# venetanji/videosd

Measured on AMD Instinct MI355X. Metric: frames/sec (whole node) + p50 per-frame latency, SD1.5 512x512 LCM 4-step, higher is better.
Workload: dtype f16 (fp32 accumulate); 1 GPU; 5 frames per launch x 4 launch lanes in flight (a stream's independent frames coalesced along GEMM M; the batch=1-per-launch figures of a --full run are fps_one_frame_per_launch and p50_latency_ms) of SD1.5 512x512 LCM 4-step img2img, every frame denoised independently, ControlNet-canny + TAESD (BASELINE configs[1], reference-faithful: the reference always runs ControlNet); frames_per_rank=414, frames_per_launch=5, launches_in_flight_per_gpu=4, kernel_launches_per_graph_replay=1430

## Files before the change

include/vsd.h:

```cpp
#ifndef VSD_H
#define VSD_H
#include <stdint.h>

#ifdef __cplusplus
extern "C" {
#endif

typedef struct vsd_ctx vsd_ctx;

enum vsd_status {
  VSD_OK = 0,
  VSD_ERR_ARG = -1,
  VSD_ERR_HIP = -2,
  VSD_ERR_NOMEM = -3,
  VSD_ERR_STATE = -4,
  VSD_PLAN_OTHER_PROGRAM = 1
};

enum vsd_act { VSD_ACT_NONE = 0, VSD_ACT_RELU = 1, VSD_ACT_SILU = 2, VSD_ACT_GEGLU = 3, VSD_ACT_QUICKGELU = 4,
               VSD_ACT_SOFTMAX = 5 ,
               VSD_ACT_GELU = 6 ,
               VSD_ACT_POST = 256  };

enum vsd_tile { VSD_TILE_128x128 = 0, VSD_TILE_128x64 = 1, VSD_TILE_64x64 = 2, VSD_TILE_64x128 = 3,
                VSD_TILE_256x128 = 4 ,
                VSD_TILE_256x64 = 5 ,
                VSD_TILE_256x256 = 6  };

enum vsd_family {
  VSD_FAM_CONV_GEMM = 0, VSD_FAM_SPLITK_REDUCE = 1, VSD_FAM_GROUPNORM = 2, VSD_FAM_LAYERNORM = 3,
  VSD_FAM_ATTENTION = 4, VSD_FAM_ELEMENTWISE = 5, VSD_FAM_COUNT = 6
};

#define VSD_VERSION 10
int vsd_version(void);
int vsd_conv_desc_size(void);

vsd_ctx* vsd_create(int device_id);
void vsd_destroy(vsd_ctx* ctx);
const char* vsd_last_error(vsd_ctx* ctx);

typedef struct vsd_conv_desc {
  const void* src0;
  const void* src1;
  int32_t c0, c1;
  int32_t hs, ws;
  int32_t hi, wi;
  int32_t ho, wo;
  int32_t ksize, stride, pad;
  const void* weight;
  int32_t n, k, kp;
  const void* bias;
  const void* rowvec;
  const void* residual;
  const void* residual2;
  int32_t ldr;
  float out_scale;
  int32_t act;
  void* out;
  int32_t ldo;
  void* out2;
  const void* add2;
  void* out_t;
  int32_t ldt, t_col0;
  int32_t tile;
  int32_t split_k;
  void* workspace;
  int32_t pipeline;
  void* rowstat_out;
  void* chanstat_out;
  void* chanstat_part;
  void* chan_counters;
  const void* ln_part;
  int32_t ln_groups;
  float ln_eps;
  const void* ln_s;
  const void* ln_t;
  void* counters;
  int32_t batch;
  int32_t t_img;
// ... 162 lines not shown
```

videosd_amd/csrc/conv_gemm.hip:

```cpp
#include "conv_kernels.h"


#ifdef VSD_CONV_PROBE
extern "C" void vsd_conv_set_probe(void* buf) { g_conv_probe = (long long*)buf; }
#endif
#ifdef VSD_WG_TIMELINE
extern "C" void vsd_wgtl_set(void* buf, int64_t words) { g_wgtl = (unsigned long long*)buf; g_wgtl_cap = (size_t)words; g_wgtl_off = 0; }
extern "C" int64_t vsd_wgtl_used(void) { return (int64_t)g_wgtl_off; }
extern "C" void vsd_cut_set(void* buf) { g_cut = (unsigned long long*)buf; }
#endif

struct ConvLaunch {
  ConvParams p;
  int BM, BN, grid, stages;
  bool halo, c64;
};

static int conv_setup(vsd_ctx* ctx, const vsd_conv_desc* d, ConvLaunch& cl, bool grouped) {
  ConvParams& p = cl.p;
  p.src0 = (const half_t*)d->src0;
  p.src1 = (const half_t*)d->src1;
  p.c0 = d->c0;
  p.c1 = d->src1 ? d->c1 : 0;
  p.cin = p.c0 + p.c1;
// ... 55 lines not shown
#endif
  p.rowstat_out = (float*)d->rowstat_out;
  p.chanstat_part = (float*)d->chanstat_part;
  p.chanstat_out = (float*)d->chanstat_out;
  p.chan_counters = (int*)d->chan_counters;
  p.ln_part = (const float*)d->ln_part;
  p.ln_groups = d->ln_groups;
  p.ln_eps = d->ln_eps;
  p.ln_s = (const float*)d->ln_s;
  p.ln_t = (const float*)d->ln_t;
  VSD_CUT_SET(p)
  const int stages = d->pipeline;
  if (stages != 0 && (stages < 3 || stages > 10)) return vsd_fail(ctx, VSD_ERR_ARG, "conv_gemm: pipeline %d (0, 3..10)", stages);
  if ((stages == 8 || stages == 9) && !p.fast)
    return vsd_fail(ctx, VSD_ERR_ARG, "conv_gemm: the eight-wave forms (pipelines 8, 9) exist for the buffer-load path only (Cin %% 64 == 0 per "
                    "source, no resize)");
  const bool c64 = stages == 10;
  const bool halo = stages == 7 || c64;

  if (!p.src0 || !p.w || !p.out) return vsd_fail(ctx, VSD_ERR_ARG, "conv_gemm: null src/weight/out");
  if (p.M <= 0 || p.N <= 0) return vsd_fail(ctx, VSD_ERR_ARG, "conv_gemm: empty problem M=%d N=%d", p.M, p.N);
  if (p.c0 % 8 || p.c1 % 8) return vsd_fail(ctx, VSD_ERR_ARG, "conv_gemm: channels must be multiples of 8 (%d,%d)", p.c0, p.c1);
  if (p.c1 && (p.c0 % 64 || p.c1 % 64)) return vsd_fail(ctx, VSD_ERR_ARG, "conv_gemm: concat sources need C %% 64 == 0");
  if (p.K != p.ksize * p.ksize * p.cin) return vsd_fail(ctx, VSD_ERR_ARG, "conv_gemm: K=%d != ks^2*Cin=%d", p.K, p.ksize * p.ksize * p.cin);
  if (p.Kp % BK || p.Kp < p.K) return vsd_fail(ctx, VSD_ERR_ARG, "conv_gemm: Kp=%d must be K rounded up to 64", p.Kp);
  if (p.ksize != 1 && p.ksize != 3) return vsd_fail(ctx, VSD_ERR_ARG, "conv_gemm: ksize %d", p.ksize);
  if (p.ldo % 8 || (p.residual && p.ldr % 8)) return vsd_fail(ctx, VSD_ERR_ARG, "conv_gemm: ld must be a multiple of 8");
  if (p.batch > 1 && p.chanstat_out) return vsd_fail(ctx, VSD_ERR_ARG, "conv_gemm: chanstat_out is per tensor, not per image (batch must be 1)");
  if (p.out_t && p.batch > 1 && (p.t_img < p.hw_out || (int64_t)p.batch * p.t_img > p.ldt))
    return vsd_fail(ctx, VSD_ERR_ARG, "conv_gemm: transposed output needs hw <= t_img and batch * t_img <= ldt");
  if (p.out2 && !p.add2) return vsd_fail(ctx, VSD_ERR_ARG, "conv_gemm: out2 without add2");
  if ((p.act & 0xff) > VSD_ACT_GELU) return vsd_fail(ctx, VSD_ERR_ARG, "conv_gemm: activation %d", p.act & 0xff);
  if ((p.act & 0xff) == VSD_ACT_GELU && (p.out_t || p.rowstat_out || p.ln_part || (p.act & VSD_ACT_POST)))
    return vsd_fail(ctx, VSD_ERR_ARG, "conv_gemm: erf GELU exists in the general epilogue walk only (no transposed output, row statistics, "
                    "fused LayerNorm or post-residual form)");
  if (p.rowstat_out && (p.N % 64 || p.out_t || (p.split_k > 1 && !d->counters)))
    return vsd_fail(ctx, VSD_ERR_ARG, "conv_gemm: rowstat_out needs N %% 64 == 0, no transposed output and the in-kernel split-K form");
  if (p.chanstat_out && (!p.chanstat_part || !p.chan_counters || p.N % 8 || p.out_t || (p.act & 0xff) == VSD_ACT_GEGLU ||
                         (p.split_k > 1 && !d->counters)))
    return vsd_fail(ctx, VSD_ERR_ARG, "conv_gemm: chanstat_out needs chanstat_part + chan_counters, N %% 8 == 0, a plain (non-transposed, "
                    "non-GEGLU) output and the in-kernel split-K form");
  if (p.ln_part && (p.ksize != 1 || !p.ln_s || !p.ln_t || p.ln_groups <= 0 || p.bias))
    return vsd_fail(ctx, VSD_ERR_ARG, "conv_gemm: fused LayerNorm needs a 1x1 layer, ln_s/ln_t and no separate bias");
  if (p.split_k > 1 && !p.ws_partial) return vsd_fail(ctx, VSD_ERR_ARG, "conv_gemm: split_k needs a workspace");
  int BM, BN;
  switch (d->tile) {
    case VSD_TILE_128x128: BM = 128; BN = 128; break;
    case VSD_TILE_128x64: BM = 128; BN = 64; break;
    case VSD_TILE_64x64: BM = 64; BN = 64; break;
    case VSD_TILE_64x128: BM = 64; BN = 128; break;
    case VSD_TILE_256x128: BM = 256; BN = 128; break;
    case VSD_TILE_256x64: BM = 256; BN = 64; break;
    case VSD_TILE_256x256: BM = 256; BN = 256; break;
    default: return vsd_fail(ctx, VSD_ERR_ARG, "conv_gemm: tile %d", d->tile);
  }
  if (halo) {
    const bool simple_epi = !p.out2 && !p.residual2 && !p.out_t && !p.rowstat_out && !p.chanstat_out && !p.ln_part &&
                            p.out_scale == 1.0f && !p.out_scale_dev &&
                            ((p.act & 0xff) == VSD_ACT_NONE || (p.act & 0xff) == VSD_ACT_RELU || (p.act & 0xff) == VSD_ACT_SILU) &&
                            !((p.act & VSD_ACT_POST) && (p.act & 0xff) != VSD_ACT_RELU);
    if (!p.halo_ok || p.ksize != 3 || p.stride != 1 || p.pad != 1 || BM < 128 || (p.N % 8 && !c64) || p.c0 % 64 || p.c1 % 64 || !simple_epi)
      return vsd_fail(ctx, VSD_ERR_ARG, "conv_gemm: the halo-patch form (pipeline 7) needs a 3x3 stride-1 conv, Cin %% 64 == 0 per "
                      "source, a 128- or 256-row tile and the plain epilogue");
  }
  if (c64) {
    const bool thin = p.N <= 8 && p.ldo == 8 && !p.residual && !(p.act & VSD_ACT_POST);
    if ((p.N != 64 && !thin) || p.cin != 64 || p.c1 != 0 || BM != 256 || BN != 64 || p.split_k != 1 || p.ldo % 8 || (size_t)p.M * p.ldo * 2 >= 0x7fffffffull)
      return vsd_fail(ctx, VSD_ERR_ARG, "conv_gemm: the persistent 64-channel form (pipeline 10) needs Cin = 64 from one source, Cout = 64 (or Cout <= 8 "
                      "with ldo = 8, no residual), tile 256x64, no split over K and an output below 2 GB");
  }
  if (BN == 256 && (stages < 8 || p.split_k != 1 || p.chanstat_out))
    return vsd_fail(ctx, VSD_ERR_ARG, "conv_gemm: the 256x256 tile exists on eight waves (pipeline 8 or 9), unsplit and without fused channel "
                    "statistics (its epilogue runs in row bands)");
  if (!halo && BM == 256 && BN != 256 && (BN != 128 || !p.fast || (stages != 3 && stages != 5 && stages < 8)))
    return vsd_fail(ctx, VSD_ERR_ARG, "conv_gemm: the 256x128 tile exists for the buffer-load path (Cin %% 64 == 0, no resize) "
                    "with the 3-stage ring (pipeline 3, 5, 8 or 9) only");
  if ((stages == 8 || stages == 9) && BM * BN < 128 * 128)
    return vsd_fail(ctx, VSD_ERR_ARG, "conv_gemm: the eight-wave forms (pipelines 8, 9) exist for tiles of 128 x 128 and larger");
  if ((p.act & 0xff) == VSD_ACT_GEGLU) {
    if (BN % 128 || p.N % 128 || p.split_k != 1 || (!p.bias && !p.ln_part) || p.out_t)
      return vsd_fail(ctx, VSD_ERR_ARG, "conv_gemm: GEGLU needs BN=128 or 256, N %% 128 == 0, bias, no split-K");
  }
  if ((p.act & 0xff) == VSD_ACT_SOFTMAX) {
    if (BN != 128 || halo || p.N % 128 || (p.split_k != 1 && !d->counters) || p.out_t || p.out2 || p.residual || p.rowstat_out || p.chanstat_out ||
        p.softmax_cols < 1 || p.softmax_cols > 128 || p.ldo % 8)
      return vsd_fail(ctx, VSD_ERR_ARG, "conv_gemm: the softmax epilogue needs BN=128, N %% 128 == 0, split-K only in the in-kernel form, a plain output and "
                      "1 <= softmax_cols <= 128");
  }
  if (p.out_t && (p.t_col0 % BN)) return vsd_fail(ctx, VSD_ERR_ARG, "conv_gemm: t_col0 must be a multiple of BN");
  p.tiles_m = halo ? p.batch * cdiv(p.ho, BM / 16) * cdiv(p.wo, 16) : cdiv(p.M, BM);
  p.tiles_n = cdiv(p.N, BN);
  const int KT = halo ? p.cin / BK : p.Kp / BK;
  if (p.split_k > KT) p.split_k = KT;
  p.kt_per_split = cdiv(KT, p.split_k);
  p.split_k = cdiv(KT, p.kt_per_split);
  if (p.split_k == 1) p.counters = nullptr;
  if (p.counters && p.tiles_m * p.tiles_n > VSD_SPLITK_MAX_TILES)
    return vsd_fail(ctx, VSD_ERR_ARG, "conv_gemm: %d tiles exceed the split-K counter buffer", p.tiles_m * p.tiles_n);
  const int grid = p.tiles_m * p.tiles_n * p.split_k;
  {
    const double a_bytes = (double)p.batch * p.img_in * p.cin * 2.0, w_bytes = (double)p.N * p.Kp * 2.0;
    const int G = p.tiles_n * p.split_k;
    const int gx = cdiv(G, 8);
    const int nslice = p.split_k < gx ? p.split_k : gx;
    const double by_w = w_bytes + a_bytes * (G < 8 ? G : 8) * nslice / (double)p.split_k;
    const double by_a = a_bytes + w_bytes * (p.tiles_m < 8 ? p.tiles_m : 8);
    const bool ok24 = p.tiles_m % 2 == 0 && G % 4 == 0, ok42 = p.tiles_m % 4 == 0 && G % 2 == 0;
    const double by_24 = ok24 ? 4.0 * a_bytes + 2.0 * w_bytes : 1e300, by_42 = ok42 ? 2.0 * a_bytes + 4.0 * w_bytes : 1e300;
    const char* force = getenv("VSD_CONV_ORDER");
    const bool no_grid = force && force[0] == '1' && force[1] == 'd';
    p.order = by_a < by_w ? 1 : 0;
    double best = by_a < by_w ? by_a : by_w;
    if (!no_grid && by_24 < best) { p.order = 2; best = by_24; }
    if (!no_grid && by_42 < best) { p.order = 3; best = by_42; }
    if (force && !no_grid) {
      const int f = atoi(force);
      if (f <= 1 || (f == 2 && ok24) || (f == 3 && ok42)) p.order = f;
// ... 116 lines not shown
```

videosd_amd/csrc/conv_halo.hip:

```cpp
#include "conv_kernels.h"

namespace {

__device__ __forceinline__ void splitk_reduce_body(const ConvParams& p) {
  VSD_CUT(VSD_CUT_REDUCE, p.cut)
  const int nch = (p.N + 7) / 8;
  const size_t total = (size_t)p.M * nch;
  const size_t slab = (size_t)p.M * p.N;
  for (size_t q = (size_t)blockIdx.x * 256 + threadIdx.x; q < total; q += (size_t)gridDim.x * 256) {
    int m = (int)(q / nch);
    int n = (int)(q - (size_t)m * nch) * 8;
    float v[8] = {0, 0, 0, 0, 0, 0, 0, 0};
    const float* s = p.ws_partial + (size_t)m * p.N + n;
    const bool full = n + 8 <= p.N;
    const bool transposed = p.out_t && n >= p.t_col0;
    const bool pre_res = full && p.residual != nullptr && !transposed;
    const bool pre_brv = false;
    const bool pre_raw = full && !p.ln_part;
    half8 rres = (half8){0, 0, 0, 0, 0, 0, 0, 0}, braw = rres, rvraw = rres;
    if (full) {
      constexpr int NB = 8;
      f32x4 lo[NB], hi[NB];
#pragma unroll
      for (int k = 0; k < NB; ++k) {
// ... 13 lines not shown
            v[4 + i] += hi[k][i];
          }
        }
      for (int k0 = NB; k0 < p.split_k; k0 += NB) {
#pragma unroll
        for (int k = 0; k < NB; ++k) {
          const int kk = k0 + k < p.split_k ? k0 + k : 0;
          lo[k] = *reinterpret_cast<const f32x4*>(s + kk * slab);
          hi[k] = *reinterpret_cast<const f32x4*>(s + kk * slab + 4);
        }
#pragma unroll
        for (int k = 0; k < NB; ++k)
          if (k0 + k < p.split_k) {
#pragma unroll
            for (int i = 0; i < 4; ++i) {
              v[i] += lo[k][i];
              v[4 + i] += hi[k][i];
            }
          }
      }
    } else {
      for (int k = 0; k < p.split_k; ++k) {
#pragma unroll
        for (int i = 0; i < 8; ++i)
          if (n + i < p.N) v[i] += s[k * slab + i];
      }
    }
    if (p.ln_part) {
      float mean, rstd;
      ln_row_stats(p, m, mean, rstd);
      ln_transform8(p, n, mean, rstd, v);
    }
    float rs = 0.f, rq = 0.f;
    const f32x4 z4 = (f32x4){0.f, 0.f, 0.f, 0.f};
    epilogue_store8(p, m, n, v, rs, rq, pre_res, rres, pre_brv, z4, z4, pre_raw, braw, rvraw);
  }
}
__global__ __launch_bounds__(256) void splitk_reduce_kernel(const ConvParams p) { splitk_reduce_body(p); }
__global__ __launch_bounds__(256) void splitk_reduce_group_kernel(const ConvGroup g) {
  const ConvParams& p = g.p[blockIdx.y];
  if (p.split_k <= 1 || p.counters) return;
  splitk_reduce_body(p);
}

template <int BN, int WMN, int NSB>
__global__ __launch_bounds__(128 * WMN) void conv_halo_kernel(const ConvParams p) {
  VSD_CUT(VSD_CUT_CONV_HALO, p.cut)
  prefetch_kernargs();
  WGTL_START()
  constexpr int NW = 2 * WMN, NT = 64 * NW;
  constexpr int BM = 64 * WMN, PW = 16, PH = 4 * WMN, HW_ = PW + 2;
  constexpr int HUSED = (PH + 2) * HW_;
  constexpr int HROWS = (HUSED + 8 * NW - 1) / (8 * NW) * (8 * NW);
  constexpr int AI = HROWS / (8 * NW), BR = BN / (8 * NW);
  static_assert(BR >= 1, "tile too narrow for this many waves");
  constexpr int TM = 64, TN = BN / 2, FM = TM / 16, FN = TN / 16;
  constexpr int BNP = BN + 4;
  constexpr int A_HALFS = HROWS * BK, B_HALFS = BN * BK;
  constexpr int STAGE_BYTES = (2 * A_HALFS + NSB * B_HALFS) * 2;
  constexpr int EPI_BYTES = BM * BNP * 4;
  constexpr int LDS_BYTES = STAGE_BYTES > EPI_BYTES ? STAGE_BYTES : EPI_BYTES;
  __shared__ __attribute__((aligned(16))) unsigned char smem[LDS_BYTES];
  half_t* Abuf = reinterpret_cast<half_t*>(smem);
  half_t* Bbuf = Abuf + 2 * A_HALFS;
  typedef __attribute__((address_space(3))) void* lds_ptr_t;
  constexpr int OOB = (int)0x80000000;

  const int tid = threadIdx.x, lane = tid & 63, wave = tid >> 6;
  const int wave_s = __builtin_amdgcn_readfirstlane(wave);
  const int wm = wave >> 1, wn = wave & 1;
  const int fr = lane & 15, fq = lane >> 4;

  int tile_m, grp;
  block_to_tile(p, blockIdx.x, tile_m, grp);
  const int split = fdiv(grp, p.fd_tiles_n);
  const int tile_n = grp - split * p.tiles_n;
  const int n0 = tile_n * BN;
  const int ppr = (p.wo + PW - 1) / PW, tpi = ((p.ho + PH - 1) / PH) * ppr;
  const int img = fdiv(tile_m, p.fd_tpi), trem = tile_m - img * tpi;
  const int prow = fdiv(trem, p.fd_ppr);
  const int y0 = prow * PH, x0 = (trem - prow * ppr) * PW;
  const int pix0 = img * p.img_in;
  const int opix0 = img * p.hw_out;
  auto row_ok = [&](int r) { return y0 + (r >> 4) < p.ho && x0 + (r & 15) < p.wo; };
  auto row_m = [&](int r) { return opix0 + (y0 + (r >> 4)) * p.wo + x0 + (r & 15); };

  const int ncb_all = p.cin / BK;
  const int cb_begin = split * p.kt_per_split;
  const int cb_end = min(ncb_all, cb_begin + p.kt_per_split);
  const int T = (cb_end - cb_begin) * 9;

  int apx[AI], alc[AI];
#pragma unroll
  for (int q = 0; q < AI; ++q) {
    const int row = 8 * (wave + NW * q) + (lane >> 3);
    const int hy = row / HW_, hx = row - hy * HW_;
    const int y = y0 - 1 + hy, x = x0 - 1 + hx;
    const bool in = row < HUSED && (unsigned)y < (unsigned)p.hi && (unsigned)x < (unsigned)p.wi;
    const int sy = (int)(((unsigned)y * p.rmul_y) >> p.rshift), sx = (int)(((unsigned)x * p.rmul_x) >> p.rshift);
    apx[q] = in ? pix0 + sy * p.ws + sx : -1;
    alc[q] = (((lane & 7) ^ (row & 7)) << 4);
  }
  int bvoff[BR];
#pragma unroll
  for (int i = 0; i < BR; ++i) {
    const int r = 8 * (wave + NW * i) + (lane >> 3);
    const int n = n0 + r;
    bvoff[i] = n < p.N ? n * p.Kp * 2 + (((lane & 7) ^ (r & 7)) << 4) : OOB;
  }
  const int anr0 = (int)((size_t)p.batch * p.img_in * p.c0 * 2), anr1 = (int)((size_t)p.batch * p.img_in * p.c1 * 2);
  const int bnr = (int)((size_t)p.N * p.Kp * 2);

#define HALO_ISSUE_A(CB_, BUF_)                                                                         \
  {                                                                                                     \
    const int ch_ = (CB_) * BK;                                                                         \
    const bool second_ = ch_ >= p.c0;                                                                   \
    const int cs2_ = (second_ ? p.c1 : p.c0) * 2;                                                       \
    const int soff_ = (second_ ? ch_ - p.c0 : ch_) * 2;                                                 \
    const __amdgpu_buffer_rsrc_t rs_ =                                                                  \
        __builtin_amdgcn_make_buffer_rsrc((void*)(second_ ? p.src1 : p.src0), 0, second_ ? anr1 : anr0, 0x00020000); \
    half_t* dst_ = Abuf + (BUF_) * A_HALFS;                                                             \
    _Pragma("unroll") for (int q = 0; q < AI; ++q) {                                                    \
      const int vo_ = apx[q] >= 0 ? __mul24(apx[q], cs2_) + alc[q] : OOB;                               \
      __builtin_amdgcn_raw_ptr_buffer_load_lds(rs_, (lds_ptr_t)(dst_ + 8 * (wave_s + NW * q) * BK), 16, vo_, soff_, 0, 0); \
    }                                                                                                   \
  }
                     \
#define HALO_ISSUE_A_PIECE(CB_, BUF_, Q_)                                                               \
  {                                                                                                     \
    const int ch_ = (CB_) * BK;                                                                         \
    const bool second_ = ch_ >= p.c0;                                                                   \
    const int cs2_ = (second_ ? p.c1 : p.c0) * 2;                                                       \
    const int soff_ = (second_ ? ch_ - p.c0 : ch_) * 2;                                                 \
    const __amdgpu_buffer_rsrc_t rs_ =                                                                  \
        __builtin_amdgcn_make_buffer_rsrc((void*)(second_ ? p.src1 : p.src0), 0, second_ ? anr1 : anr0, 0x00020000); \
    half_t* dst_ = Abuf + (BUF_) * A_HALFS;                                                             \
    int apx_ = apx[0], alc_ = alc[0];                                                                   \
    _Pragma("unroll") for (int q = 1; q < AI; ++q)                                                      \
      if (q == (Q_)) {                                                                                  \
        apx_ = apx[q];                                                                                  \
        alc_ = alc[q];                                                                                  \
      }                                                                                                 \
    const int vo_ = apx_ >= 0 ? __mul24(apx_, cs2_) + alc_ : OOB;                                       \
    __builtin_amdgcn_raw_ptr_buffer_load_lds(rs_, (lds_ptr_t)(dst_ + 8 * (wave_s + NW * (Q_)) * BK), 16, vo_, soff_, 0, 0); \
  }
#define HALO_ISSUE_B(TAP_, CB_, SLOT_)                                                                  \
  {                                                                                                     \
    const int soff_ = ((TAP_) * p.cin + (CB_) * BK) * 2;                                                \
    const __amdgpu_buffer_rsrc_t rsb_ = __builtin_amdgcn_make_buffer_rsrc((void*)p.w, 0, bnr, 0x00020000); \
    half_t* dst_ = Bbuf + (SLOT_) * B_HALFS;                                                            \
    _Pragma("unroll") for (int i = 0; i < BR; ++i) {                                                    \
      const int bv_ = bvoff[i] + 0;                                                                     \
      __builtin_amdgcn_raw_ptr_buffer_load_lds(rsb_, (lds_ptr_t)(dst_ + 8 * (wave_s + NW * i) * BK), 16, bv_, soff_, 0, 0); \
    }                                                                                                   \
  }

#ifdef VSD_CONV_PROBE
  long long pacc[8] = {0, 0, 0, 0, 0, 0, 0, 0};
  long long plast = __builtin_readcyclecounter();
#endif
  f32x4 acc[FM][FN];
#pragma unroll
  for (int i = 0; i < FM; ++i)
#pragma unroll
    for (int j = 0; j < FN; ++j) acc[i][j] = (f32x4){0.f, 0.f, 0.f, 0.f};

  int hr0[FM];
#pragma unroll
  for (int i = 0; i < FM; ++i) hr0[i] = (wm * (TM / PW) + i) * HW_ + fr;

  if (T > 0) {
    HALO_ISSUE_A(cb_begin, 0)
#pragma unroll
    for (int st = 0; st < NSB - 1; ++st)
      if (st < T) HALO_ISSUE_B(st % 9, cb_begin + st / 9, st)
  }
  constexpr int LEAD = NSB - 1;
  int tap = 0, cb = cb_begin, slot = 0;
  int tap2 = LEAD % 9, cb2 = cb_begin + LEAD / 9;
  int hist = 0;
  CPROBE(0)
  for (int t = 0; t < T; ++t) {
    const int later_b = min(LEAD - 1, T - 1 - t) * BR;
    const int nwait = later_b + __builtin_popcount(hist & ((1 << LEAD) - 1));
    if (nwait >= (LEAD - 1) * BR + LEAD) asm volatile("s_waitcnt vmcnt(%0)" ::"n"((LEAD - 1) * BR + LEAD) : "memory");
    else if (nwait >= (LEAD - 1) * BR + 1) asm volatile("s_waitcnt vmcnt(%0)" ::"n"((LEAD - 1) * BR + 1) : "memory");
    else if (nwait >= (LEAD - 1) * BR) asm volatile("s_waitcnt vmcnt(%0)" ::"n"((LEAD - 1) * BR) : "memory");
    else if (nwait >= BR) asm volatile("s_waitcnt vmcnt(%0)" ::"n"(BR) : "memory");
    else asm volatile("s_waitcnt vmcnt(0)" ::: "memory");
    CPROBE(1)
    __builtin_amdgcn_s_barrier();
    CPROBE(2)
    if (t + LEAD < T) {
      int ns = slot + LEAD;
      if (ns >= NSB) ns -= NSB;
      HALO_ISSUE_B(tap2, cb2, ns)
    }
    hist <<= 1;
    if (tap < AI && cb + 1 < cb_end) {
      HALO_ISSUE_A_PIECE(cb + 1, (cb + 1 - cb_begin) & 1, tap)
      hist |= 1;
    }
    CPROBE(3)
    const half_t* a = Abuf + ((cb - cb_begin) & 1) * A_HALFS;
    const half_t* b = Bbuf + slot * B_HALFS;
    const int ky = tap / 3, kx = tap - ky * 3;
    const int toff = ky * HW_ + kx;
    half8 af[2][FM], bf[2][FN];
#pragma unroll
    for (int i = 0; i < FM; ++i) {
      const int hr = hr0[i] + toff;
      const half_t* row = a + hr * BK;
      const int sw = hr & 7;
      af[0][i] = *reinterpret_cast<const half8*>(row + ((fq ^ sw) << 3));
      af[1][i] = *reinterpret_cast<const half8*>(row + (((4 + fq) ^ sw) << 3));
    }
#pragma unroll
    for (int j = 0; j < FN; ++j) {
      const int r = wn * TN + j * 16 + fr;
      const half_t* row = b + r * BK;
      bf[0][j] = *reinterpret_cast<const half8*>(row + ((fq ^ (r & 7)) << 3));
      bf[1][j] = *reinterpret_cast<const half8*>(row + (((4 + fq) ^ (r & 7)) << 3));
    }
#pragma unroll
    for (int ks = 0; ks < 2; ++ks)
#pragma unroll
      for (int i = 0; i < FM; ++i)
#pragma unroll
        for (int j = 0; j < FN; ++j) acc[i][j] = __builtin_amdgcn_mfma_f32_16x16x32_f16(af[ks][i], bf[ks][j], acc[i][j], 0, 0, 0);
    CPROBE(4)
    if (++slot == NSB) slot = 0;
    if (++tap == 9) { tap = 0; ++cb; }
    if (++tap2 == 9) { tap2 = 0; ++cb2; }
  }
#undef HALO_ISSUE_A
#undef HALO_ISSUE_A_PIECE
#undef HALO_ISSUE_B
  __syncthreads();
  WGTL_LOOP()

  constexpr int CH = BN / 8;
  constexpr int NIT = BM * CH / NT;
  half8 rpre[NIT];
  float brv[8], brv2[8];
  const int pre_n = n0 + (tid % CH) * 8;
  const bool ncol_ok = pre_n + 8 <= p.N;
#pragma unroll
  for (int i = 0; i < 8; ++i) brv[i] = brv2[i] = 0.f;
  if (p.split_k == 1) {
    if (ncol_ok && p.bias) {
      half8 v = *reinterpret_cast<const half8*>(p.bias + pre_n);
#pragma unroll
      for (int i = 0; i < 8; ++i) brv[i] += (float)v[i];
    }
    if (ncol_ok && p.rowvec) {
      half8 v = *reinterpret_cast<const half8*>(p.rowvec + pre_n);
#pragma unroll
      for (int i = 0; i < 8; ++i) brv[i] += (float)v[i];
    }
    if (p.residual) {
#pragma unroll
      for (int j = 0; j < NIT; ++j) {
        const int q = tid + j * NT;
        const int r = q / CH;
        rpre[j] = *reinterpret_cast<const half8*>(p.residual + (ncol_ok && row_ok(r) ? (size_t)row_m(r) * p.ldr + pre_n : 0));
      }
    }
  }
  float* Cs = reinterpret_cast<float*>(smem);
#pragma unroll
  for (int i = 0; i < FM; ++i)
#pragma unroll
    for (int j = 0; j < FN; ++j) {
      const int col = wn * TN + j * 16 + fr;
      const int row = wm * TM + i * 16 + fq * 4;
#pragma unroll
      for (int r = 0; r < 4; ++r) Cs[(row + r) * BNP + col] = acc[i][j][r];
    }
  __syncthreads();
  CPROBE(5)
  bool from_slabs = false;
  if (p.split_k > 1) {
    float* slab = p.ws_partial + (size_t)split * p.M * p.N;
    const bool wt = p.counters != nullptr;
    __amdgpu_buffer_rsrc_t rsrc = __builtin_amdgcn_make_buffer_rsrc(
        slab, 0, (int)min((size_t)p.M * p.N * sizeof(float), (size_t)0x7fffffff), 0x00020000);
#pragma unroll
    for (int j = 0; j < NIT; ++j) {
      const int q = tid + j * NT;
      const int r = q / CH, c8 = (q - r * CH) * 8;
      const int n = n0 + c8;
      if (n + 8 <= p.N && row_ok(r)) {
        const float* sp = Cs + r * BNP + c8;
        if (wt) {
          const int off = (int)(((size_t)row_m(r) * p.N + n) * sizeof(float));
          __builtin_amdgcn_raw_buffer_store_b128(*reinterpret_cast<const u32x4*>(sp), rsrc, off, 0, 16);
          __builtin_amdgcn_raw_buffer_store_b128(*reinterpret_cast<const u32x4*>(sp + 4), rsrc, off + 16, 0, 16);
        } else {
          float* d = slab + (size_t)row_m(r) * p.N + n;
          *reinterpret_cast<f32x4*>(d) = *reinterpret_cast<const f32x4*>(sp);
          *reinterpret_cast<f32x4*>(d + 4) = *reinterpret_cast<const f32x4*>(sp + 4);
        }
      }
    }
    if (!p.counters) { WGTL_END(1) return; }
    asm volatile("s_waitcnt vmcnt(0)" ::: "memory");
    __syncthreads();
    int* lastflag = reinterpret_cast<int*>(smem);
    if (tid == 0) {
      int* cnt = p.counters + tile_n * p.tiles_m + tile_m;
      const int ticket = __hip_atomic_fetch_add(cnt, 1, __ATOMIC_RELAXED, __HIP_MEMORY_SCOPE_AGENT);
      const int last = ticket == p.split_k - 1;
      if (last) {
        __builtin_amdgcn_fence(__ATOMIC_ACQUIRE, "agent");
        asm volatile("s_waitcnt vmcnt(0)" ::: "memory");
        __hip_atomic_store(cnt, 0, __ATOMIC_RELAXED, __HIP_MEMORY_SCOPE_AGENT);
      }
      *lastflag = last;
    }
    __syncthreads();
    if (!*lastflag) { WGTL_END(1) return; }
    from_slabs = true;
    if (ncol_ok && p.bias) {
      half8 v = *reinterpret_cast<const half8*>(p.bias + pre_n);
#pragma unroll
      for (int i = 0; i < 8; ++i) brv[i] += (float)v[i];
    }
    if (ncol_ok && p.rowvec) {
      half8 v = *reinterpret_cast<const half8*>(p.rowvec + pre_n);
#pragma unroll
      for (int i = 0; i < 8; ++i) brv2[i] = (float)v[i];
    }
    if (p.residual) {
#pragma unroll
      for (int j = 0; j < NIT; ++j) {
        const int q = tid + j * NT;
        const int r = q / CH;
        rpre[j] = *reinterpret_cast<const half8*>(p.residual + (ncol_ok && row_ok(r) ? (size_t)row_m(r) * p.ldr + pre_n : 0));
      }
    }
  }
  const int act = p.act & 0xff;
  const bool post = (p.act & VSD_ACT_POST) != 0;
  auto finish = [&](auto act_tag) __attribute__((always_inline)) {
    constexpr int ACT = decltype(act_tag)::value;
#pragma unroll
    for (int j = 0; j < NIT; ++j) {
      const int q = tid + j * NT;
      const int r = q / CH, c8 = (q - r * CH) * 8;
      const int n = n0 + c8;
      if (n + 8 <= p.N && row_ok(r)) {
        f32x4 lo, hi;
        if (from_slabs) {
          lo = hi = (f32x4){0.f, 0.f, 0.f, 0.f};
          const float* sp = p.ws_partial + (size_t)row_m(r) * p.N + n;
          const size_t slab_sz = (size_t)p.M * p.N;
          constexpr int NB = 8;
          for (int k0 = 0; k0 < p.split_k; k0 += NB) {
            f32x4 a[NB], b[NB];
#pragma unroll
            for (int k = 0; k < NB; ++k) {
              const int kk = k0 + k < p.split_k ? k0 + k : 0;
              a[k] = *reinterpret_cast<const f32x4*>(sp + kk * slab_sz);
              b[k] = *reinterpret_cast<const f32x4*>(sp + kk * slab_sz + 4);
            }
#pragma unroll
            for (int k = 0; k < NB; ++k)
              if (k0 + k < p.split_k) {
#pragma unroll
                for (int i = 0; i < 4; ++i) {
                  lo[i] += a[k][i];
                  hi[i] += b[k][i];
                }
              }
          }
        } else {
          lo = *reinterpret_cast<const f32x4*>(Cs + r * BNP + c8);
          hi = *reinterpret_cast<const f32x4*>(Cs + r * BNP + c8 + 4);
        }
        const float v[8] = {lo[0], lo[1], lo[2], lo[3], hi[0], hi[1], hi[2], hi[3]};
        half8 o;
#pragma unroll
        for (int i = 0; i < 8; ++i) {
          float x = (v[i] + brv[i]) + brv2[i];
          if (ACT == 1) x = fmaxf(x, 0.f);
          if (ACT == 2) x = silu_f(x);
          if (p.residual) x += (float)rpre[j][i];
          if (ACT == 3) x = fmaxf(x, 0.f);
          o[i] = (half_t)x;
        }
        VSD_OUT_STORE8(p.out + (size_t)row_m(r) * p.ldo + n, o);
      }
    }
  };
  if (act == VSD_ACT_RELU && post) finish(std::integral_constant<int, 3>{});
  else if (act == VSD_ACT_RELU) finish(std::integral_constant<int, 1>{});
  else if (act == VSD_ACT_SILU) finish(std::integral_constant<int, 2>{});
  else finish(std::integral_constant<int, 0>{});
  CPROBE(6)
  CPROBE_OUT()
  WGTL_END(1)
}

}

void vsd_launch_conv_halo(const ConvParams& p, int BM, int BN, int grid, hipStream_t s) {
  if (BM == 256 && BN == 128) hipLaunchKernelGGL((conv_halo_kernel<128, 4, 3>), dim3(grid), dim3(512), 0, s, p);
  else if (BM == 256) hipLaunchKernelGGL((conv_halo_kernel<64, 4, 3>), dim3(grid), dim3(512), 0, s, p);
  else if (BN == 128) hipLaunchKernelGGL((conv_halo_kernel<128, 2, 3>), dim3(grid), dim3(256), 0, s, p);
  else hipLaunchKernelGGL((conv_halo_kernel<64, 2, 3>), dim3(grid), dim3(256), 0, s, p);
}

void vsd_launch_splitk_reduce(const ConvParams& p, int grid, hipStream_t s) {
  hipLaunchKernelGGL(splitk_reduce_kernel, dim3(grid), dim3(256), 0, s, p);
}
void vsd_launch_splitk_reduce_group(const ConvGroup& g, int grid, hipStream_t s) {
  hipLaunchKernelGGL(splitk_reduce_group_kernel, dim3(grid, g.n), dim3(256), 0, s, g);
}
```

videosd_amd/lib.py:

```python
import ctypes as C
import os

HERE = os.path.dirname(os.path.abspath(__file__))
LIB_PATH = os.environ.get("VSD_LIB") or os.path.join(HERE, "libvsd.so")

VERSION = 10
ACT_NONE, ACT_RELU, ACT_SILU, ACT_GEGLU, ACT_QUICKGELU, ACT_SOFTMAX, ACT_GELU = range(7)
ACT_POST = 256
SPLITK_MAX_TILES = 16384
POOL_STREAMS = 4
CONV_GROUP_MAX = 8
RESAMPLE_MAX_SIDE = 16384
MERGE_SEG_MAX = 16
TILE_128x128, TILE_128x64, TILE_64x64, TILE_64x128, TILE_256x128, TILE_256x64, TILE_256x256 = range(7)
TILE_DIMS = {TILE_128x128: (128, 128), TILE_128x64: (128, 64), TILE_64x64: (64, 64), TILE_64x128: (64, 128),
             TILE_256x128: (256, 128), TILE_256x64: (256, 64), TILE_256x256: (256, 256)}
FAMILIES = ["conv_gemm", "splitk_reduce", "groupnorm", "layernorm", "attention", "elementwise"]


class ConvDesc(C.Structure):
    _fields_ = [
        ("src0", C.c_void_p), ("src1", C.c_void_p),
        ("c0", C.c_int32), ("c1", C.c_int32),
        ("hs", C.c_int32), ("ws", C.c_int32),
        ("hi", C.c_int32), ("wi", C.c_int32),
        ("ho", C.c_int32), ("wo", C.c_int32),
        ("ksize", C.c_int32), ("stride", C.c_int32), ("pad", C.c_int32),
        ("weight", C.c_void_p),
        ("n", C.c_int32), ("k", C.c_int32), ("kp", C.c_int32),
        ("bias", C.c_void_p), ("rowvec", C.c_void_p), ("residual", C.c_void_p), ("residual2", C.c_void_p),
        ("ldr", C.c_int32),
        ("out_scale", C.c_float),
        ("act", C.c_int32),
        ("out", C.c_void_p), ("ldo", C.c_int32),
        ("out2", C.c_void_p), ("add2", C.c_void_p),
        ("out_t", C.c_void_p), ("ldt", C.c_int32), ("t_col0", C.c_int32),
        ("tile", C.c_int32), ("split_k", C.c_int32),
        ("workspace", C.c_void_p),
        ("pipeline", C.c_int32),
        ("rowstat_out", C.c_void_p), ("chanstat_out", C.c_void_p), ("chanstat_part", C.c_void_p),
        ("chan_counters", C.c_void_p), ("ln_part", C.c_void_p), ("ln_groups", C.c_int32), ("ln_eps", C.c_float),
        ("ln_s", C.c_void_p), ("ln_t", C.c_void_p),
        ("counters", C.c_void_p),
        ("batch", C.c_int32), ("t_img", C.c_int32),
        ("out_scale_dev", C.c_void_p),
        ("softmax_cols", C.c_int32),
    ]


SIGNATURES = {
    "vsd_version": (C.c_int, []),
    "vsd_conv_desc_size": (C.c_int, []),
    "vsd_xattn_fold": (C.c_int, [C.c_void_p, C.c_void_p, C.c_int, C.c_void_p, C.c_int, C.c_int, C.c_void_p, C.c_void_p, C.c_void_p,
                                C.c_void_p, C.c_int, C.c_int, C.c_float, C.c_void_p, C.c_void_p, C.c_void_p, C.c_void_p, C.c_void_p]),
    "vsd_create": (C.c_void_p, [C.c_int]),
    "vsd_destroy": (None, [C.c_void_p]),
    "vsd_last_error": (C.c_char_p, [C.c_void_p]),
    "vsd_conv_gemm": (C.c_int, [C.c_void_p, C.POINTER(ConvDesc), C.c_void_p]),
    "vsd_conv_gemm_group": (C.c_int, [C.c_void_p, C.POINTER(ConvDesc), C.c_int, C.c_void_p]),
    "vsd_pair_begin": (C.c_int, [C.c_void_p]),
    "vsd_pair_join": (C.c_int, [C.c_void_p]),
    "vsd_pair_end": (C.c_int, [C.c_void_p, C.POINTER(C.c_int)]),
    "vsd_tail_a": (C.c_int, [C.c_void_p] * 3 + [C.c_int] + [C.c_void_p] * 5 + [C.c_float] + [C.c_void_p] * 3),
    "vsd_tail_b": (C.c_int, [C.c_void_p] * 4 + [C.c_int] + [C.c_void_p] * 5 + [C.c_float] + [C.c_void_p] * 6),
    "vsd_groupnorm_workspace_bytes": (C.c_int64, [C.c_int, C.c_int, C.c_int]),
    "vsd_groupnorm": (C.c_int, [C.c_void_p, C.c_void_p, C.c_void_p, C.c_int, C.c_int, C.c_int, C.c_int, C.c_float,
                                C.c_void_p, C.c_void_p, C.c_int, C.c_void_p, C.c_void_p, C.c_void_p]),
    "vsd_layernorm": (C.c_int, [C.c_void_p, C.c_void_p, C.c_int, C.c_int, C.c_void_p, C.c_void_p, C.c_float,
                                C.c_void_p, C.c_void_p]),
# ... 149 lines not shown
```

videosd_amd/ops.py:

```python
import ctypes as C
import math
import time
from dataclasses import dataclass
from typing import Optional

import torch

from . import lib as L
from .packing import PackedConv

import os as _os

POISON = bool(_os.environ.get("VSD_POISON"))


@dataclass(frozen=True)
class Geom:
    hs: int
    ws: int
    hi: int
    wi: int
    ho: int
    wo: int
    ksize: int = 1
# ... 244 lines not shown
            self._ws[key] = cur
        if self.allocator is not None and cur.numel() != max(nbytes, 256):
            with torch.cuda.stream(self.stream):
                cur = self._ws[key] = self.allocator(max(nbytes, 256))
        return cur

    def synchronize(self):
        for st in reversed(self.streams):
            st.synchronize()

    def upload(self, dst: torch.Tensor, src_cpu: torch.Tensor):
        with torch.cuda.stream(self.stream):
            dst.copy_(src_cpu.view(dst.shape), non_blocking=src_cpu.is_pinned())

    def download(self, src: torch.Tensor) -> torch.Tensor:
        with torch.cuda.stream(self.stream):
            out = src.to("cpu", non_blocking=False)
        return out

    def download_into(self, dst_cpu: torch.Tensor, src: torch.Tensor):
        with torch.cuda.stream(self.stream):
            dst_cpu.view(src.shape).copy_(src, non_blocking=True)
        self.stream.synchronize()

    def conv(self, src0, src1, g: Geom, w: PackedConv, out, *, ldo=None, c0=None, c1=0, rowvec=None, residual=None,
             residual2=None, ldr=None, out_scale=1.0, act=L.ACT_NONE, out2=None, add2=None, out_t=None, ldt=0,
             t_col0=0, tile=None, split_k=None, workspace=None, pipeline=None, rowstat_out=None, ln_part=None,
             ln_eps=1e-5, chanstat_out=None, t_img=0, out_scale_dev=None, softmax_cols=0, _desc_only=False):
        m = g.m
        c0 = c0 if c0 is not None else (w.cin - c1)
        if w.geglu:
            act = L.ACT_GEGLU
        key = self.conv_key(g, w, t_col0, self.epilogue_class(w, rowstat_out, ln_part, chanstat_out, residual2, out2, out_scale_dev, out_scale, act))
        inkernel = self.inkernel_splitk
        if tile is None:
            if key not in self.tile_override and key[-1] == 1 and key[:-1] + (0,) in self.tile_override:
                key = key[:-1] + (0,)
            if key in self.tile_override:
                tile, split_k, inkernel, pipeline = self.tile_override[key]
            else:
                tile, sk = choose_tile(m, w.n, w.kp, w.geglu or w.tile128, t_col0 if out_t is not None else 0)
                split_k = sk if split_k is None else split_k
        split_k = split_k or 1
        if w.tile128:
            inkernel = True
        if pipeline == 10 and (self.no_c64 or out_scale_dev is not None or
                               not self._c64_call_ok(g, w, c1, act, out_scale, residual, residual2, out2, out_t, rowstat_out, chanstat_out, ln_part,
                                                     ldo if ldo is not None else w.n_out)):
            pipeline, tile, split_k = (7, L.TILE_256x64, 1) if w.n % 8 == 0 else (3, L.TILE_64x64, 1)
        if pipeline == 7 and (self.no_halo or out_scale_dev is not None or
                              not self._halo_call_ok(g, w, c1, act, out_scale, residual2, out2, out_t, rowstat_out,
                                                     chanstat_out, ln_part)):
            pipeline = 3
            tile = {L.TILE_256x128: L.TILE_128x128, L.TILE_256x64: L.TILE_128x64}.get(tile, tile)
            inkernel = True
        d = L.ConvDesc()
        d.src0, d.src1 = self._p(src0), self._p(src1)
        d.c0, d.c1 = c0, c1
        d.hs, d.ws, d.hi, d.wi, d.ho, d.wo = g.hs, g.ws, g.hi, g.wi, g.ho, g.wo
        d.ksize, d.stride, d.pad = g.ksize, g.stride, g.pad
        d.weight = self._p(w.weight)
        d.n, d.k, d.kp = w.n, w.k, w.kp
        d.bias = self._p(w.bias)
        if ln_part is not None:
            if w.ln_s is None:
                raise RuntimeError("conv: ln_part given but the weights were not packed with pack_linear_ln")
            d.ln_part, d.ln_groups, d.ln_eps = self._p(ln_part), ln_part.shape[1], ln_eps
            d.ln_s, d.ln_t = self._p(w.ln_s), self._p(w.ln_t)
        d.rowstat_out = self._p(rowstat_out)
        if chanstat_out is not None:
            d.chanstat_out = self._p(chanstat_out)
            d.chanstat_part = self._p(self.workspace("chanpart", (-(-m // 64)) * w.n * 8))
            d.chan_counters = self._p(self._counter_set(self._chan_counters, 4096))
        d.rowvec = self._p(rowvec)
        d.residual, d.residual2 = self._p(residual), self._p(residual2)
        d.ldr = ldr if ldr is not None else w.n_out
        d.out_scale = out_scale
        d.out_scale_dev = self._p(out_scale_dev)
        d.softmax_cols = softmax_cols
        d.act = act
        d.out = self._p(out)
        d.ldo = ldo if ldo is not None else w.n_out
        d.out2, d.add2 = self._p(out2), self._p(add2)
        d.out_t, d.ldt, d.t_col0 = self._p(out_t), ldt, t_col0
        d.batch, d.t_img = g.batch, t_img
        d.tile, d.split_k = tile, split_k
        d.pipeline = self.default_pipeline if pipeline is None else pipeline
        if split_k > 1:
            ws = workspace if workspace is not None else self.workspace("splitk", split_k * m * w.n * 4)
            d.workspace = self._p(ws)
            if inkernel:
                d.counters = self._p(self._counter_set(self._counters, L.SPLITK_MAX_TILES))
        elif workspace is not None:
            d.workspace = self._p(workspace)
        if _desc_only:
            return d
        self.ctx.call("vsd_conv_gemm", C.byref(d), self.s)

    GROUP_FORMS = [(L.TILE_64x64, 3), (L.TILE_64x64, 5), (L.TILE_64x128, 3), (L.TILE_64x128, 5), (L.TILE_128x64, 3), (L.TILE_128x64, 5),
                   (L.TILE_128x128, 3), (L.TILE_128x128, 5), (L.TILE_128x128, 8), (L.TILE_128x128, 9)]
    GROUP_ALONE = -1
    OWN_SPLIT = "own"

    def own_splits(self, calls):
        out = []
        for a, kw in calls:
            kw = {k: v for k, v in kw.items() if k not in ("tile", "split_k", "pipeline")}
# ... 159 lines not shown
        return (g.m, w.n, w.kp, g.ksize, g.stride, g.hi != g.hs or g.wi != g.ws, w.geglu, t_col0, int(epi), int(self.tune_mode))

    def conv_key_of(self, g: Geom, w: PackedConv, kwargs: dict):
        return self.conv_key(g, w, kwargs.get("t_col0", 0), self.epilogue_class(
            w, kwargs.get("rowstat_out"), kwargs.get("ln_part"), kwargs.get("chanstat_out"), kwargs.get("residual2"), kwargs.get("out2"),
            kwargs.get("out_scale_dev"), kwargs.get("out_scale", 1.0), kwargs.get("act", L.ACT_NONE)))

    def tune_conv(self, args, kwargs, reps: int = 12):
        g, w = args[2], args[3]
        t_col0 = kwargs.get("t_col0", 0)
        key = self.conv_key_of(g, w, kwargs)
        kt = w.kp // 64
        wide = w.geglu or w.tile128
        tiles = [L.TILE_128x128, L.TILE_64x128] if wide else [L.TILE_128x128, L.TILE_128x64, L.TILE_64x128, L.TILE_64x64]
        big_path = w.cin % 64 == 0 and (kwargs.get("c1", 0) or 0) % 64 == 0 and (g.hi, g.wi) == (g.hs, g.ws)
        big_ok = big_path and g.m >= 1024
        if big_ok:
            tiles = tiles + [L.TILE_256x128]
        huge_ok = (big_path and g.m >= 1024 and w.n >= 512 and not w.tile128 and kwargs.get("out_t") is None and
                   kwargs.get("chanstat_out") is None and not self.no_w8 and self.tune_mode == 1)

        plain_epi = all(kwargs.get(k) is None for k in ("out2", "residual2", "out_t", "rowstat_out", "chanstat_out", "ln_part"))
        act = kwargs.get("act", L.ACT_NONE)
        halo_ok = (not wide and g.ksize == 3 and g.stride == 1 and w.cin % 64 == 0 and
                   (kwargs.get("c1", 0) or 0) % 64 == 0 and w.n % 8 == 0 and plain_epi and
                   kwargs.get("out_scale", 1.0) == 1.0 and act in (L.ACT_NONE, L.ACT_RELU, L.ACT_SILU, L.ACT_RELU | L.ACT_POST))
        cands = [(L.TILE_256x256, 1, False, pl) for pl in (8, 9)] if huge_ok else []
        for t in tiles:
            bm, bn = L.TILE_DIMS[t]
            if kwargs.get("out_t") is not None and t_col0 % bn:
                continue
            blocks = -(-g.m // bm) * -(-w.n // bn)
            w8 = (8, 9) if big_path and bm * bn >= 128 * 128 and not self.no_w8 and self.tune_mode == 1 else ()
            for pl in ((3, 5) if t == L.TILE_256x128 else (0, 3, 4, 5, 6)) + w8:
                cands.append((t, 1, False, pl))
            if halo_ok and bm == 128:
                hblocks = g.batch * -(-g.ho // 8) * -(-g.wo // 16) * -(-w.n // bn)
                for sp in (1, 2, 3, 4, 5, 6, 8, 10, 12, 16, 20):
                    if sp > w.cin // 64 or (sp > 1 and hblocks * sp > 1536):
                        break
                    cands.append((t, sp, False, 7))
                    if sp > 1 and hblocks <= L.SPLITK_MAX_TILES:
                        cands.append((t, sp, True, 7))
            if w.geglu or blocks >= 384:
                continue
            for sp in (2, 3, 4, 6, 8, 12, 16, 24):
                if sp > kt // 2 or blocks * sp > 1536:
                    break
                for pl in ((3, 5) if t == L.TILE_256x128 else (0, 3, 5)) + w8:
                    if kwargs.get("rowstat_out") is None and kwargs.get("chanstat_out") is None and not w.tile128:
                        cands.append((t, sp, False, pl))
                    cands.append((t, sp, True, pl))
        if halo_ok:
            for t in (L.TILE_256x128, L.TILE_256x64):
                bn = L.TILE_DIMS[t][1]
                hblocks = g.batch * -(-g.ho // 16) * -(-g.wo // 16) * -(-w.n // bn)
                for sp in (1, 2, 3, 4, 5, 6, 8, 10, 12, 16, 20):
                    if sp > w.cin // 64 or (sp > 1 and hblocks * sp > 1536):
                        break
                    cands.append((t, sp, False, 7))
                    if sp > 1 and hblocks <= L.SPLITK_MAX_TILES:
                        cands.append((t, sp, True, 7))
        if not self.no_c64 and not wide and kwargs.get("out_scale_dev") is None and self._c64_call_ok(
                g, w, kwargs.get("c1", 0) or 0, act, kwargs.get("out_scale", 1.0), kwargs.get("residual"), kwargs.get("residual2"), kwargs.get("out2"),
                kwargs.get("out_t"), kwargs.get("rowstat_out"), kwargs.get("chanstat_out"), kwargs.get("ln_part"),
                kwargs.get("ldo") if kwargs.get("ldo") is not None else w.n_out):
            cands.append((L.TILE_256x64, 1, False, 10))
        kw = {k: v for k, v in kwargs.items() if k not in ("tile", "split_k", "pipeline")}
        table = []
        saved = self.tile_override.pop(key, None)
        if self.tune_mode == 1:
            alone = self._time_candidates(args, kw, cands, reps)
            if not alone:
                raise RuntimeError("tune_conv: no candidate ran")
            cut = 2.5 * alone[0][0]
            short = [(t, sp, ink, pl) for (us, t, sp, ink, pl) in alone if us <= cut or (t == L.TILE_256x256 and us <= 6.0 * alone[0][0])]
            table = self._time_candidates_on_lanes(args, kw, short, reps) or alone
            self.inkernel_splitk = True
            best = table[0]
            self.tile_override[key] = (best[1], best[2], best[3], best[4])
            return best, table
        last_error = None
        for (t, sp, ink, pl) in cands:
            self.inkernel_splitk = ink
            try:
                for _ in range(2):
                    self.conv(*args, tile=t, split_k=sp, pipeline=pl, **kw)
                best_us = 1e30
                for _trial in range(2):
                    e0, e1 = torch.cuda.Event(enable_timing=True), torch.cuda.Event(enable_timing=True)
                    e0.record(self.stream)
                    for _ in range(reps):
                        self.conv(*args, tile=t, split_k=sp, pipeline=pl, **kw)
                    e1.record(self.stream)
                    e1.synchronize()
                    best_us = min(best_us, e0.elapsed_time(e1) / reps * 1e3)
                table.append((best_us, t, sp, ink, pl))
            except RuntimeError as e:
                last_error = e
                continue
        self.inkernel_splitk = True
        if not table:
            raise RuntimeError(f"tune_conv: no candidate ran for M={g.m} N={w.n} K={w.k} ksize={g.ksize}: {last_error}")
        table.sort()
        best = table[0]
        if best[2] > 1 and not best[3] and self.one_launch_bias_us > 0:
            for cand in table[1:]:
                if cand[0] > best[0] + self.one_launch_bias_us:
                    break
# ... 321 lines not shown
```

Before: 147.9 frames/s.

## Add 160-column halo conv tiles for channel counts divisible by 160

Adds 128x160 and 256x160 tile variants to the halo-patch 3x3 conv kernel and offers them to the autotuner for layers whose output channels are a multiple of 160 (SD1.5's 320/640/1280). The B-tile load handles a remainder row group spread over a subset of waves. The epilogue handles thread counts that do not divide the column-chunk count, and rotates columns when the padded epilogue tile would overflow LDS. The aim is to cover those channel counts without partial 128-column tiles wasting MFMA work and blocks. The cost is more template instances and extra epilogue index arithmetic.

New measurement: 150.3 frames/s, median of 6. 1.02x the previous value.

```diff
diff --git a/include/vsd.h b/include/vsd.h
--- a/include/vsd.h
+++ b/include/vsd.h
@@ -25,7 +25,8 @@
 enum vsd_tile { VSD_TILE_128x128 = 0, VSD_TILE_128x64 = 1, VSD_TILE_64x64 = 2, VSD_TILE_64x128 = 3,
                 VSD_TILE_256x128 = 4 ,
                 VSD_TILE_256x64 = 5 ,
-                VSD_TILE_256x256 = 6  };
+                VSD_TILE_256x256 = 6 ,
+                VSD_TILE_128x160 = 7, VSD_TILE_256x160 = 8  };
 
 enum vsd_family {
   VSD_FAM_CONV_GEMM = 0, VSD_FAM_SPLITK_REDUCE = 1, VSD_FAM_GROUPNORM = 2, VSD_FAM_LAYERNORM = 3,
diff --git a/videosd_amd/csrc/conv_gemm.hip b/videosd_amd/csrc/conv_gemm.hip
--- a/videosd_amd/csrc/conv_gemm.hip
+++ b/videosd_amd/csrc/conv_gemm.hip
@@ -131,6 +131,8 @@
     case VSD_TILE_256x128: BM = 256; BN = 128; break;
     case VSD_TILE_256x64: BM = 256; BN = 64; break;
     case VSD_TILE_256x256: BM = 256; BN = 256; break;
+    case VSD_TILE_128x160: BM = 128; BN = 160; break;
+    case VSD_TILE_256x160: BM = 256; BN = 160; break;
     default: return vsd_fail(ctx, VSD_ERR_ARG, "conv_gemm: tile %d", d->tile);
   }
   if (halo) {
@@ -142,6 +144,8 @@
       return vsd_fail(ctx, VSD_ERR_ARG, "conv_gemm: the halo-patch form (pipeline 7) needs a 3x3 stride-1 conv, Cin %% 64 == 0 per "
                       "source, a 128- or 256-row tile and the plain epilogue");
   }
+  if (BN == 160 && !(halo && !c64))
+    return vsd_fail(ctx, VSD_ERR_ARG, "conv_gemm: the 160-column tiles exist in the halo-patch form (pipeline 7) only");
   if (c64) {
     const bool thin = p.N <= 8 && p.ldo == 8 && !p.residual && !(p.act & VSD_ACT_POST);
     if ((p.N != 64 && !thin) || p.cin != 64 || p.c1 != 0 || BM != 256 || BN != 64 || p.split_k != 1 || p.ldo % 8 || (size_t)p.M * p.ldo * 2 >= 0x7fffffffull)
diff --git a/videosd_amd/csrc/conv_halo.hip b/videosd_amd/csrc/conv_halo.hip
--- a/videosd_amd/csrc/conv_halo.hip
+++ b/videosd_amd/csrc/conv_halo.hip
@@ -89,14 +89,20 @@
   constexpr int BM = 64 * WMN, PW = 16, PH = 4 * WMN, HW_ = PW + 2;
   constexpr int HUSED = (PH + 2) * HW_;
   constexpr int HROWS = (HUSED + 8 * NW - 1) / (8 * NW) * (8 * NW);
-  constexpr int AI = HROWS / (8 * NW), BR = BN / (8 * NW);
-  static_assert(BR >= 1, "tile too narrow for this many waves");
+  constexpr int AI = HROWS / (8 * NW);
+  constexpr int BRF = BN / (8 * NW), BREM = BN % (8 * NW);
+  constexpr int BR = BRF + (BREM ? 1 : 0), BREMW = BREM ? BREM / 8 : 1;
+  static_assert(BRF >= 1 && BREM % 8 == 0 && NW % BREMW == 0, "tile too narrow for this many waves");
   constexpr int TM = 64, TN = BN / 2, FM = TM / 16, FN = TN / 16;
-  constexpr int BNP = BN + 4;
+  constexpr int LDS_CU = 160 * 1024;
+  constexpr bool ROT = BM * (BN + 4) * 4 > LDS_CU;
+  constexpr int BNP = ROT ? BN : BN + 4;
+  static_assert(!ROT || BN % 16 == 0, "the rotation moves whole 16-column fragments");
   constexpr int A_HALFS = HROWS * BK, B_HALFS = BN * BK;
   constexpr int STAGE_BYTES = (2 * A_HALFS + NSB * B_HALFS) * 2;
   constexpr int EPI_BYTES = BM * BNP * 4;
   constexpr int LDS_BYTES = STAGE_BYTES > EPI_BYTES ? STAGE_BYTES : EPI_BYTES;
+  static_assert(LDS_BYTES <= LDS_CU, "stage ring / epilogue tile larger than a CU's LDS");
   __shared__ __attribute__((aligned(16))) unsigned char smem[LDS_BYTES];
   half_t* Abuf = reinterpret_cast<half_t*>(smem);
   half_t* Bbuf = Abuf + 2 * A_HALFS;
@@ -141,7 +147,7 @@
   int bvoff[BR];
 #pragma unroll
   for (int i = 0; i < BR; ++i) {
-    const int r = 8 * (wave + NW * i) + (lane >> 3);
+    const int r = 8 * ((BREM && i == BRF ? wave % BREMW : wave) + NW * i) + (lane >> 3);
     const int n = n0 + r;
     bvoff[i] = n < p.N ? n * p.Kp * 2 + (((lane & 7) ^ (r & 7)) << 4) : OOB;
   }
@@ -188,7 +194,8 @@
     half_t* dst_ = Bbuf + (SLOT_) * B_HALFS;                                                            \
     _Pragma("unroll") for (int i = 0; i < BR; ++i) {                                                    \
       const int bv_ = bvoff[i] + 0;                                                                     \
-      __builtin_amdgcn_raw_ptr_buffer_load_lds(rsb_, (lds_ptr_t)(dst_ + 8 * (wave_s + NW * i) * BK), 16, bv_, soff_, 0, 0); \
+      const int wv_ = BREM && i == BRF ? wave_s % BREMW : wave_s;                                       \
+      __builtin_amdgcn_raw_ptr_buffer_load_lds(rsb_, (lds_ptr_t)(dst_ + 8 * (wv_ + NW * i) * BK), 16, bv_, soff_, 0, 0); \
     }                                                                                                   \
   }
 
@@ -277,7 +284,11 @@
   WGTL_LOOP()
 
   constexpr int CH = BN / 8;
-  constexpr int NIT = BM * CH / NT;
+  constexpr bool EVEN = NT % CH == 0;
+  constexpr int NTE = NT / CH * CH;
+  constexpr int NIT = (BM * CH + NTE - 1) / NTE;
+  auto q_ok = [&](int q) { return EVEN || (tid < NTE && q < BM * CH); };
+  auto cs_col = [&](int r, int c) { return ROT ? (c + 16 * ((r >> 2) & 3)) % BN : c; };
   half8 rpre[NIT];
   float brv[8], brv2[8];
   const int pre_n = n0 + (tid % CH) * 8;
@@ -298,9 +309,9 @@
     if (p.residual) {
 #pragma unroll
       for (int j = 0; j < NIT; ++j) {
-        const int q = tid + j * NT;
+        const int q = tid + j * NTE;
         const int r = q / CH;
-        rpre[j] = *reinterpret_cast<const half8*>(p.residual + (ncol_ok && row_ok(r) ? (size_t)row_m(r) * p.ldr + pre_n : 0));
+        rpre[j] = *reinterpret_cast<const half8*>(p.residual + (q_ok(q) && ncol_ok && row_ok(r) ? (size_t)row_m(r) * p.ldr + pre_n : 0));
       }
     }
   }
@@ -312,7 +323,7 @@
       const int col = wn * TN + j * 16 + fr;
       const int row = wm * TM + i * 16 + fq * 4;
 #pragma unroll
-      for (int r = 0; r < 4; ++r) Cs[(row + r) * BNP + col] = acc[i][j][r];
+      for (int r = 0; r < 4; ++r) Cs[(row + r) * BNP + cs_col(row + r, col)] = acc[i][j][r];
     }
   __syncthreads();
   CPROBE(5)
@@ -324,11 +335,11 @@
         slab, 0, (int)min((size_t)p.M * p.N * sizeof(float), (size_t)0x7fffffff), 0x00020000);
 #pragma unroll
     for (int j = 0; j < NIT; ++j) {
-      const int q = tid + j * NT;
+      const int q = tid + j * NTE;
       const int r = q / CH, c8 = (q - r * CH) * 8;
       const int n = n0 + c8;
-      if (n + 8 <= p.N && row_ok(r)) {
-        const float* sp = Cs + r * BNP + c8;
+      if (q_ok(q) && n + 8 <= p.N && row_ok(r)) {
+        const float* sp = Cs + r * BNP + cs_col(r, c8);
         if (wt) {
           const int off = (int)(((size_t)row_m(r) * p.N + n) * sizeof(float));
           __builtin_amdgcn_raw_buffer_store_b128(*reinterpret_cast<const u32x4*>(sp), rsrc, off, 0, 16);
@@ -371,9 +382,9 @@
     if (p.residual) {
 #pragma unroll
       for (int j = 0; j < NIT; ++j) {
-        const int q = tid + j * NT;
+        const int q = tid + j * NTE;
         const int r = q / CH;
-        rpre[j] = *reinterpret_cast<const half8*>(p.residual + (ncol_ok && row_ok(r) ? (size_t)row_m(r) * p.ldr + pre_n : 0));
+        rpre[j] = *reinterpret_cast<const half8*>(p.residual + (q_ok(q) && ncol_ok && row_ok(r) ? (size_t)row_m(r) * p.ldr + pre_n : 0));
       }
     }
   }
@@ -383,10 +394,10 @@
     constexpr int ACT = decltype(act_tag)::value;
 #pragma unroll
     for (int j = 0; j < NIT; ++j) {
-      const int q = tid + j * NT;
+      const int q = tid + j * NTE;
       const int r = q / CH, c8 = (q - r * CH) * 8;
       const int n = n0 + c8;
-      if (n + 8 <= p.N && row_ok(r)) {
+      if (q_ok(q) && n + 8 <= p.N && row_ok(r)) {
         f32x4 lo, hi;
         if (from_slabs) {
           lo = hi = (f32x4){0.f, 0.f, 0.f, 0.f};
@@ -412,8 +423,8 @@
               }
           }
         } else {
-          lo = *reinterpret_cast<const f32x4*>(Cs + r * BNP + c8);
-          hi = *reinterpret_cast<const f32x4*>(Cs + r * BNP + c8 + 4);
+          lo = *reinterpret_cast<const f32x4*>(Cs + r * BNP + cs_col(r, c8));
+          hi = *reinterpret_cast<const f32x4*>(Cs + r * BNP + cs_col(r, c8) + 4);
         }
         const float v[8] = {lo[0], lo[1], lo[2], lo[3], hi[0], hi[1], hi[2], hi[3]};
         half8 o;
@@ -442,7 +453,9 @@
 }
 
 void vsd_launch_conv_halo(const ConvParams& p, int BM, int BN, int grid, hipStream_t s) {
-  if (BM == 256 && BN == 128) hipLaunchKernelGGL((conv_halo_kernel<128, 4, 3>), dim3(grid), dim3(512), 0, s, p);
+  if (BM == 256 && BN == 160) hipLaunchKernelGGL((conv_halo_kernel<160, 4, 3>), dim3(grid), dim3(512), 0, s, p);
+  else if (BN == 160) hipLaunchKernelGGL((conv_halo_kernel<160, 2, 3>), dim3(grid), dim3(256), 0, s, p);
+  else if (BM == 256 && BN == 128) hipLaunchKernelGGL((conv_halo_kernel<128, 4, 3>), dim3(grid), dim3(512), 0, s, p);
   else if (BM == 256) hipLaunchKernelGGL((conv_halo_kernel<64, 4, 3>), dim3(grid), dim3(512), 0, s, p);
   else if (BN == 128) hipLaunchKernelGGL((conv_halo_kernel<128, 2, 3>), dim3(grid), dim3(256), 0, s, p);
   else hipLaunchKernelGGL((conv_halo_kernel<64, 2, 3>), dim3(grid), dim3(256), 0, s, p);
diff --git a/videosd_amd/lib.py b/videosd_amd/lib.py
--- a/videosd_amd/lib.py
+++ b/videosd_amd/lib.py
@@ -12,9 +12,10 @@
 CONV_GROUP_MAX = 8
 RESAMPLE_MAX_SIDE = 16384
 MERGE_SEG_MAX = 16
-TILE_128x128, TILE_128x64, TILE_64x64, TILE_64x128, TILE_256x128, TILE_256x64, TILE_256x256 = range(7)
+TILE_128x128, TILE_128x64, TILE_64x64, TILE_64x128, TILE_256x128, TILE_256x64, TILE_256x256, TILE_128x160, TILE_256x160 = range(9)
 TILE_DIMS = {TILE_128x128: (128, 128), TILE_128x64: (128, 64), TILE_64x64: (64, 64), TILE_64x128: (64, 128),
-             TILE_256x128: (256, 128), TILE_256x64: (256, 64), TILE_256x256: (256, 256)}
+             TILE_256x128: (256, 128), TILE_256x64: (256, 64), TILE_256x256: (256, 256), TILE_128x160: (128, 160),
+             TILE_256x160: (256, 160)}
 FAMILIES = ["conv_gemm", "splitk_reduce", "groupnorm", "layernorm", "attention", "elementwise"]
 
 
diff --git a/videosd_amd/ops.py b/videosd_amd/ops.py
--- a/videosd_amd/ops.py
+++ b/videosd_amd/ops.py
@@ -320,7 +320,8 @@
                               not self._halo_call_ok(g, w, c1, act, out_scale, residual2, out2, out_t, rowstat_out,
                                                      chanstat_out, ln_part)):
             pipeline = 3
-            tile = {L.TILE_256x128: L.TILE_128x128, L.TILE_256x64: L.TILE_128x64}.get(tile, tile)
+            tile = {L.TILE_256x128: L.TILE_128x128, L.TILE_256x64: L.TILE_128x64, L.TILE_128x160: L.TILE_128x128,
+                    L.TILE_256x160: L.TILE_128x128}.get(tile, tile)
             inkernel = True
         d = L.ConvDesc()
         d.src0, d.src1 = self._p(src0), self._p(src1)
@@ -586,9 +587,10 @@
                         cands.append((t, sp, False, pl))
                     cands.append((t, sp, True, pl))
         if halo_ok:
-            for t in (L.TILE_256x128, L.TILE_256x64):
-                bn = L.TILE_DIMS[t][1]
-                hblocks = g.batch * -(-g.ho // 16) * -(-g.wo // 16) * -(-w.n // bn)
+            n160 = (L.TILE_128x160, L.TILE_256x160) if w.n % 160 == 0 else ()
+            for t in (L.TILE_256x128, L.TILE_256x64) + n160:
+                bm, bn = L.TILE_DIMS[t]
+                hblocks = g.batch * -(-g.ho // (bm // 16)) * -(-g.wo // 16) * -(-w.n // bn)
                 for sp in (1, 2, 3, 4, 5, 6, 8, 10, 12, 16, 20):
                     if sp > w.cin // 64 or (sp > 1 and hblocks * sp > 1536):
                         break
```
